# AliBahri94/GM3D

Hardware: AMD Instinct MI355X
Metric: point-clouds/sec pretrain step (N=1024,G=64) (higher is better)
Workload: dtype bf16

## Files before the change

### gm3d_amd/_capi.py

```python
import ctypes
import os

_HERE = os.path.dirname(os.path.abspath(__file__))
LIB_PATH = os.environ.get("GM3D_HIP_LIB") or os.path.join(_HERE, "lib", "libgm3d_hip.so")

GM3D_OK, GM3D_EINVAL, GM3D_EUNSUPPORTED, GM3D_ELAUNCH = 0, -1, -2, -3
GM3D_F32, GM3D_BF16 = 0, 1

_vp, _i, _f = ctypes.c_void_p, ctypes.c_int, ctypes.c_float

SIGNATURES = {
    "gm3d_abi_version": [],
    "gm3d_strerror": [_i],
    "gm3d_fps": [_vp, _i, _i, _i, _vp, _vp, _vp],
    "gm3d_gather_points": [_vp, _vp, _i, _i, _i, _i, _vp, _vp],
    "gm3d_gather_points_grad": [_vp, _vp, _i, _i, _i, _i, _vp, _vp],
    "gm3d_knn": [_vp, _vp, _i, _i, _i, _i, _vp, _vp, _vp],
    "gm3d_knn_group": [_vp, _vp, _i, _i, _i, _i, _vp, _vp, _vp, _vp],
    "gm3d_chamfer_fwd": [_vp, _vp, _i, _i, _i, _vp, _vp, _vp, _vp, _vp],
    "gm3d_chamfer_bwd": [_vp, _vp, _vp, _vp, _vp, _vp, _i, _i, _i, _vp, _vp, _vp],
    "gm3d_patch_chamfer_loss_fwd": [_vp, ctypes.c_longlong, _vp, _vp, ctypes.c_longlong, _i, _i, _i, _vp, _vp, _vp, _vp, _i, _vp],
    "gm3d_patch_chamfer_loss_bwd": [_vp, ctypes.c_longlong, _vp, _vp, ctypes.c_longlong, _vp, _vp, _vp, _i, _i, _i, _vp, _i, _vp],
    "gm3d_attention_fwd": [_vp, _vp, _vp, _i, _i, _i, _f, _i, _vp],
    "gm3d_attention_qkv_fwd": [_vp, _vp, _vp, _vp, _vp, _i, _i, _i, _i, _f, _i, _vp],
    "gm3d_attention_bwd": [_vp, _vp, _vp, _vp, _vp, _i, _i, _i, _f, _i, _vp],
    "gm3d_ln_plain_partial_rows": [_i],
    "gm3d_ln_plain_fwd": [_vp, _vp, _vp, _f, _vp, _vp, _vp, _i, _i, _i, _vp],
    "gm3d_ln_plain_bwd": [_vp, _vp, _vp, _vp, _vp, _vp, _vp, _i, _i, _i, _vp],
    "gm3d_residual_ln_fwd": [_vp, _vp, _vp, _vp, _i, _vp, _vp, _vp, _f, _vp, _vp, _vp, _vp, _i, _i, _i, _vp],
    "gm3d_residual_ln_bwd": [_vp, _vp, _vp, _vp, _vp, _vp, _vp, _i, _vp, _vp, _vp, _vp, _vp, _i, _i, _i, _vp],
    "gm3d_ln_partial_rows": [_i],
    "gm3d_colsum_finish": [_vp, _i, _i, _i, _vp, _i, _vp],
    "gm3d_colsum_finish_batched": [_vp, _i, ctypes.c_longlong, _i, _i, _i, _vp, _i, _vp],
    "gm3d_bias_gelu_fwd": [_vp, _vp, _vp, _i, _i, _i, _vp],
    "gm3d_bias_gelu_bwd": [_vp, _vp, _vp, _vp, _vp, _i, _i, _i, _vp],
    "gm3d_gelu_partial_rows": [_i],
    "gm3d_embed_partial_rows": [_i, _i, _i],
    "gm3d_moments3": [_vp, _i, _vp, _vp],
    "gm3d_pn_layer1_fwd": [_vp, _vp, _vp, _vp, _i, _i, _i, _vp],
    "gm3d_group_max_fwd": [_vp, _vp, _vp, _vp, _i, _i, _i, _i, _vp],
    "gm3d_group_max_bwd": [_vp, _vp, _vp, _i, _i, _i, _i, _vp],
    "gm3d_bn_bcast_stats": [_vp, _vp, _i, _i, _i, _vp, _i, _vp],
    "gm3d_bn_bcast_apply_relu": [_vp, _vp, _vp, _vp, _vp, _i, _i, _i, _f, _i, _vp],
    "gm3d_bn_bcast_bwd_stats": [_vp, _vp, _vp, _vp, _vp, _vp, _vp, _i, _i, _i, _vp, _f, _i, _vp],
    "gm3d_bn_bcast_bwd_apply": [_vp, _vp, _vp, _vp, _vp, _vp, _vp, _vp, _vp, _vp, _vp, _i, _i, _i, _f, _i, _vp],
    "gm3d_head_fold": [_vp, _vp, _i, _i, _vp, _vp, _vp, _i, _vp],
    "gm3d_head_rowdot": [_vp, _vp, _vp, _i, _i, _vp, _i, _vp],
    "gm3d_head_fold_bwd": [_vp, _vp, _i, _i, _i, _vp, _vp, _vp],
    "gm3d_head_outer": [_vp, _vp, _i, _i, _vp, _i, _vp],
    "gm3d_scale_translate": [_vp, _vp, _f, _f, _f, _i, _i, _vp],
    "gm3d_group_select_maps": [_vp, _i, _i, _i, _i, _vp, _vp, _vp],
    "gm3d_bn_bcast_apply_relu_sel": [_vp, _vp, _vp, _vp, _vp, _vp, _i, _i, _i, _f, _i, _vp],
    "gm3d_bn_bcast_bwd_stats_sel": [_vp, _vp, _vp, _vp, _vp, _vp, _vp, _vp, _i, _i, _i, _vp, _f, _i, _vp],
    "gm3d_bn_bcast_bwd_apply_sel": [_vp, _vp, _vp, _vp, _vp, _vp, _vp, _vp, _vp, _vp, _vp, _vp, _i, _i, _i, _f, _i, _vp],
    "gm3d_lin3_gelu_fwd": [_vp, _vp, _vp, _vp, _i, _i, _i, _vp],
    "gm3d_lin3_gelu_bwd": [_vp, _vp, _vp, _vp, _i, _i, _vp, _i, _vp],
    "gm3d_lin3_finish": [_vp, _i, _i, _vp, _vp, _vp],
    "gm3d_rank_loss": [_vp, _vp, _i, _i, _vp, _vp, _vp],
    "gm3d_rank_loss_tail": [_vp, _i, _vp, _i, _i, _vp, _vp, _vp, _vp, _vp],
    "gm3d_rank_loss_tail_bwd": [_vp, _vp, _vp, _i, _i, _i, _vp, _vp],
    "gm3d_ema_counters": [_vp, _vp, _i, _f, _f, _vp],
    "gm3d_drop_path_scales": [_vp, _vp, _i, _i, _vp, _vp],
    "gm3d_pad_cols": [_vp, ctypes.c_longlong, _i, _i, _vp, _i, _i, _vp],
    "gm3d_patch_chamfer_loss_bwd_full": [_vp, ctypes.c_longlong, _vp, _vp, ctypes.c_longlong, _vp, _vp, _vp, _i, _i, _i, _i, _vp, _i, _vp],
    "gm3d_mask_select_b": [_vp, _vp, _i, _i, _i, _i, _vp, _vp, _vp, _vp, _i, _vp],
    "gm3d_pn1_bwd_finalize": [_vp, _vp, _vp, _vp, _vp, _vp, _vp, _vp, _i, _vp],
    "gm3d_gemm_tn_bf16": [_vp, _vp, _vp, _vp, _i, _i, _i, _i, _i, _i, _vp],
    "gm3d_gemm_tn_bf16_gelu": [_vp, _vp, _vp, _vp, _vp, _i, _i, _i, _i, _i, _i, _i, _vp],
    "gm3d_gemm_tn_bf16_pool": [_vp, _vp, _vp, _vp, _vp, _vp, _i, _i, _i, _i, _i, _i, _i, _i, _vp],
    "gm3d_gemm_tn_bf16_gelu_bwd": [_vp, _vp, _vp, _vp, _vp, _vp, _i, _i, _i, _i, _i, _i, _i, _vp],
    "gm3d_gemm_tn_bf16_res": [_vp, _vp, _vp, _vp, _vp, _i, _vp, _vp, _vp, _vp, _i, _i, _i, _i, _i, _i, _vp],
    "gm3d_gemm_tn_bf16_lna": [_vp, _vp, _vp, _vp, _f, _vp, _vp, _vp, _vp, _vp, _vp, _vp, _i, _i, _i, _i, _i, _i, _i, _vp],
    "gm3d_gemm_tile_rows": [_i],
    "gm3d_gemm_tn_bf16_ring": [_vp, _vp, _vp, _vp, _i, _i, _i, _i, _i, _i, _i, _vp],
    "gm3d_gemm_tn_bf16_ws": [_vp, _vp, _vp, _vp, _i, _i, _i, _i, _i, _i, _vp],
    "gm3d_gemm_tn_bf16_ws_pool": [_vp, _vp, _vp, _vp, _vp, _vp, _i, _i, _i, _i, _i, _i, _i, _i, _vp],
    "gm3d_gemm_ws_supported": [_i, _i, _i],
    "gm3d_gemm_tn_bf16_ws_poolg": [_vp, _vp, _vp, _vp, _vp, _vp, _i, _i, _i, _i, _i, _i, _i, _i, _i, _vp],
    "gm3d_gemm_nt_bf16_sum": [_vp, _vp, _vp, _vp, _vp, _i, _i, _i, _i, _i, _i, _i, ctypes.c_longlong, ctypes.c_longlong, ctypes.c_longlong, _i, _vp],
    "gm3d_gemm_nt_tiles": [_i, _i],
    "gm3d_gemm_nt_bf16_multi": [_i] + [_vp] * 14 + [_vp],
    "gm3d_gemm_tn_bf16_ws_bn_apply": [_vp, _vp, _vp, _vp, _vp, _f, _vp, _i, _i, _i, _i, _i, _i, _i, _vp],
    "gm3d_gemm_tn_bf16_ws_bn_stats": [_vp, _vp, _vp, _vp, _vp, _i, _i, _i, _i, _i, _i, _i, _vp],
    "gm3d_gemm_ws_stats_rows": [_i, _i, _i],
    "gm3d_gemm_tn_bf16_ws_bn_apply_g": [_vp, _vp, _vp, _vp, _vp, _f, _vp, _i, _i, _i, _i, _i, _i, _i, _i, _vp],
    "gm3d_gemm_tn_bf16_ws_bn_stats_g": [_vp, _vp, _vp, _vp, _vp, _i, _i, _i, _i, _i, _i, _i, _i, _vp],
    "gm3d_gemm_tn_bf16_ring96": [_vp, _vp, _vp, _vp, _i, _i, _i, _i, _i, _i, _i, _vp],
    "gm3d_gemm_tn_bf16_dma": [_vp, _vp, _vp, _vp, _i, _i, _i, _i, _i, _i, _i, _vp],
    "gm3d_gemm_tn_bf16_dma_gelu_bwd": [_vp, _vp, _vp, _vp, _vp, _vp, _i, _i, _i, _i, _i, _i, _i, _i, _vp],
    "gm3d_gemm_tn_bf16_dma_gelu": [_vp, _vp, _vp, _vp, _vp, _i, _i, _i, _i, _i, _i, _i, _i, _vp],
    "gm3d_transpose_bf16_batched": [_vp, _vp, _i, _i, _i, ctypes.c_longlong, _vp],
    "gm3d_transpose_bf16_multi": [_i, _vp, _vp, _vp, _vp, _vp, _vp, _vp],
    "gm3d_token_assemble_fwd": [_vp, _vp, _vp, _i, _i, _i, _i, _vp, _vp, _vp, _i, _vp],
    "gm3d_token_assemble_bwd": [_vp, _vp, _vp, _vp, _i, _i, _i, _i, _vp, _vp, _i, _vp],
    "gm3d_sum_few_rows": [_vp, _i, _i, ctypes.c_longlong, _vp, _vp],
    "gm3d_gemm_nt_bf16": [_vp, _vp, _vp, _i, _i, _i, _i, _i, _i, _i, ctypes.c_longlong, ctypes.c_longlong, ctypes.c_longlong, _i,
                          ctypes.c_longlong, _vp],
    "gm3d_gemm_nt_bf16_big": [_vp, _vp, _vp, _i, _i, _i, _i, _i, _i, _i, ctypes.c_longlong, ctypes.c_longlong, ctypes.c_longlong, _i,
                              ctypes.c_longlong, _vp],
    "gm3d_gemm_nt_splits": [_i, _i, _i, _i],
    "gm3d_radius_mask_bits": [_vp, _vp, _f, _i, _i, _vp, _vp],
    "gm3d_radius_mask_bits_m": [_vp, _vp, _i, _f, _i, _i, _vp, _vp],
    "gm3d_attention_masked_fwd": [_vp, _vp, _vp, _vp, _i, _i, _i, _i, _f, _i, _vp],
    "gm3d_attention_masked_bwd": [_vp, _vp, _vp, _vp, _vp, _vp, _i, _i, _i, _i, _f, _i, _vp],
    "gm3d_mask_select": [_vp, _vp, _i, _i, _i, _i, _vp, _vp, _vp, _i, _vp],
    "gm3d_bn_finalize": [_vp, ctypes.c_double, _vp, _vp, _f, _f, _vp, _vp, _vp, _vp, _vp, _vp, _vp, _i, _i, _vp],
    "gm3d_pn1_finalize": [_vp, ctypes.c_double, _vp, _vp, _vp, _vp, _f, _f, _vp, _vp, _vp, _vp, _vp, _vp, _vp, _vp, _vp, _i, _i, _vp],
    "gm3d_flat_partial_rows": [ctypes.c_longlong],
    "gm3d_adamw_ema_flat_step": [_vp, _vp, _vp, _vp, _vp, _vp, _vp, ctypes.c_longlong, ctypes.c_longlong, _vp, _f, _f, _f, _f,
                                 _vp, _f, _vp, _vp, _vp, _vp],
    "gm3d_adamw_ema_flat_step_lrd": [_vp, _vp, _vp, _vp, _vp, _vp, _vp, ctypes.c_longlong, ctypes.c_longlong, _vp, _vp, _f, _f,
                                     _f, _f, _vp, _f, _vp, _vp, _vp, _vp],
    "gm3d_group_scatter_add": [_vp, _vp, _vp, _i, _i, _i, _vp, _i, _vp],
    "gm3d_pn_layer1_bwd_stats": [_vp, _vp, _vp, _vp, _vp, _vp, _vp, _vp, _i, _i, _vp, _i, _vp],
    "gm3d_colsum_finish_f64": [_vp, _i, _i, _i, _vp, _vp],
    "gm3d_colsum_partial": [_vp, _i, _i, _vp, _i, _vp],
    "gm3d_gather_inverse": [_vp, _i, _i, _i, _vp, _vp, _vp],
    "gm3d_gather_rows_bwd": [_vp, _vp, _vp, _vp, _i, _i, _i, _i, _i, _vp],
    "gm3d_add_ln_fwd": [_vp, _vp, _vp, _vp, _i, _vp, _vp, _vp, _f, _vp, _vp, _vp, _vp, _i, _i, _i, _vp],
    "gm3d_add_ln_bwd": [_vp, _vp, _vp, _vp, _vp, _vp, _vp, _i, _vp, _vp, _vp, _i, _i, _i, _i, _vp],
    "gm3d_add_ln_bwd_acc": [_vp, _vp, _vp, _vp, _vp, _vp, _vp, _i, _vp, _vp, _vp, _i, _vp, _i, _i, _i, _i, _vp],
    "gm3d_partition_visible": [_vp, _i, _i, _i, _vp, _vp, _vp, _vp, _vp, _vp, _vp],
    "gm3d_select_rows": [_vp, _vp, _vp, _vp, _i, _i, _i, _i, _i, _vp],
    "gm3d_back_project": [_vp, _vp, _i, _i, _i, _i, _vp, _vp],
    "gm3d_interp3_fwd": [_vp, _vp, _vp, _vp, _vp, _i, _i, _i, _i, _i, _i, _vp],
    "gm3d_gather_rows_bwd_w": [_vp, _i, _i, _i, _vp, _vp, _vp, _vp, _i, _i, _i, _i, _i, _vp],
    "gm3d_where_rows": [_vp, _i, _vp, _vp, _i, _vp, ctypes.c_longlong, _i, _i, _vp],
    "gm3d_take_rows": [_vp, _vp, _vp, _i, _i, _i, _i, _i, _vp],
    "gm3d_colsum_partial_w": [_vp, _vp, _i, _i, _vp, _i, _vp],
    "gm3d_gemm_tn_bf16_dma_pool": [_vp, _vp, _vp, _vp, _vp, _vp, _i, _i, _i, _i, _i, _i, _i, _i, _i, _i, _vp],
    "gm3d_gemm_tn_bf16_dmaw": [_vp, _vp, _vp, _vp, _i, _i, _i, _i, _i, _i, _i, _i, _vp],
    "gm3d_vote_sample": [_vp, _vp, _vp, _vp, _vp, _i, _i, _i, _i, _i, _vp, _vp],
    "gm3d_cls_tail_vote": [_vp, _i, _i, _i, _i] + [_vp] * 14 + [_i, _f, _vp, _vp, _vp, _vp, _vp, _i, _vp],
    "gm3d_cls_tail_fwd": [_vp, _i, _i, _i, _i] + [_vp] * 10 + [_i] + [_vp] * 6 + [_f, _f, _i] + [_vp] * 8 + [_i, _vp],
    "gm3d_cls_tail_bwd": [_i, _i, _i, _i] + [_vp] * 7 + [_i, _i] + [_vp] * 21 + [_i, _vp],
    "gm3d_cls_tail_vote_pool": [_vp, _i, _i, _i, _i, _i] + [_vp] * 14 + [_i, _f, _vp, _vp, _vp, _vp, _vp, _vp, _i, _vp],
    "gm3d_svm_gram": [_vp, _i, _i, _vp, _vp],
    "gm3d_svm_smo": [_vp, _i, _i, _vp, ctypes.c_double, ctypes.c_double, ctypes.c_longlong, _vp, _vp, _vp, _vp, _vp],
    "gm3d_svm_weights": [_vp, _i, _i, _i, _vp, _vp, _vp, _vp],
    "gm3d_svm_predict": [_vp, _i, _i, _i, _vp, _vp, _vp, _vp, _vp, _vp],
}


class Gm3dError(RuntimeError):
    pass


def _load():
    if not os.path.exists(LIB_PATH):
        raise ImportError(
            "gm3d_amd: %s not found. Build it with `python -m gm3d_amd.build` "
            "(hipcc, --offload-arch=gfx950). There is no CPU fallback." % LIB_PATH)
    lib = ctypes.CDLL(LIB_PATH)
    for name, argtypes in SIGNATURES.items():
        fn = getattr(lib, name)
        fn.argtypes = argtypes
        fn.restype = ctypes.c_char_p if name == "gm3d_strerror" else ctypes.c_int
    return lib


lib = _load()


def check(rc, what):
    if rc != GM3D_OK:
        raise Gm3dError("%s failed: %s (code %d)" % (what, lib.gm3d_strerror(rc).decode(), rc))
```

### gm3d_amd/build.py

```python
import glob
import os
import subprocess
import sys

HERE = os.path.dirname(os.path.abspath(__file__))
CSRC = os.path.join(HERE, "csrc")
OUT_DIR = os.path.join(HERE, "lib")
LIB = os.path.join(OUT_DIR, "libgm3d_hip.so")
ARCH = "gfx950"

SOURCES = {
    "capi.hip": [],
    "fps.hip": ["-ffp-contract=off"],
    "knn.hip": ["-ffp-contract=off"],
    "chamfer.hip": ["-ffp-contract=off"],
    "attention.hip": [],
    "rowops.hip": [],
    "embed.hip": [],
    "optim.hip": [],
    "gemm.hip": [],
    "gemm_nt.hip": [],
    "gemm_ring.hip": [],
    "gemm_dma.hip": [],
    "gemm_ws.hip": [],
    "gather.hip": [],
    "attention_masked.hip": [],
    "vote.hip": [],
    "cls_tail.hip": [],
    "svm.hip": ["-ffp-contract=off"],
}
COMMON = ["--offload-arch=" + ARCH, "-O3", "-fPIC", "-std=c++17", "-Wall", "-Wno-unused-function"]


def _stale(target, deps):
    if not os.path.exists(target):
        return True
    t = os.path.getmtime(target)
    return any(os.path.getmtime(d) > t for d in deps)


def build(force=False, verbose=False):
    hipcc = os.environ.get("HIPCC", "/opt/rocm/bin/hipcc")
    os.makedirs(OUT_DIR, exist_ok=True)
    hdrs = sorted(glob.glob(os.path.join(CSRC, "*.hpp"))) + [os.path.join(HERE, "..", "include", "gm3d.h")]
    objs = []
    for src, extra in SOURCES.items():
        s = os.path.join(CSRC, src)
        o = os.path.join(OUT_DIR, src.replace(".hip", ".o"))
        if force or _stale(o, [s] + hdrs):
            cmd = [hipcc] + COMMON + extra + ["-c", s, "-o", o]
            if verbose:
                print(" ".join(cmd))
            subprocess.check_call(cmd)
        objs.append(o)
    if force or _stale(LIB, objs):
        cmd = [hipcc, "--offload-arch=" + ARCH, "-shared", "-fPIC", "-o", LIB] + objs
        if verbose:
            print(" ".join(cmd))
        subprocess.check_call(cmd)
    return LIB


if __name__ == "__main__":
    print(build(force="--force" in sys.argv, verbose=True))
```

### gm3d_amd/embed.py

```python
import torch

from ._capi import lib
from .fused import weight_cache, LNC
from . import gemm
from .ops import _launch, _ptr, _stream, _DT

SPLITK = 64


def _finish(partial, nrows, ncols, pitch=None):
    out = torch.empty(ncols, dtype=torch.float32, device=partial.device)
    _launch("gm3d_colsum_finish", {"rows": nrows, "cols": ncols}, lib.gm3d_colsum_finish, _ptr(partial), nrows,
            pitch or ncols, ncols, _ptr(out), 0, _stream())
    return out


def colsum(m, adt):
    R, C = m.shape
    nrows = lib.gm3d_embed_partial_rows(2, R, C)
    partial = torch.empty(nrows, C, dtype=torch.float32, device=m.device)
    _launch("gm3d_colsum_partial", {"R": R, "C": C, "dtype": str(m.dtype)}, lib.gm3d_colsum_partial, _ptr(m), R, C,
            _ptr(partial), _DT[m.dtype], _stream())
    return _finish(partial, nrows, C)


def splitk_wgrad(dy, x):
    R, N = dy.shape
    K = x.shape[1]
    from . import gemm
    if dy.is_contiguous() and x.is_contiguous() and gemm.wgrad_supported(dy.unsqueeze(0), x.unsqueeze(0)):
        return gemm.wgrad_nt(dy.unsqueeze(0), x.unsqueeze(0))[0]
    if (N % 128 and N < 128 and dy.is_contiguous() and x.is_contiguous() and dy.dtype == torch.bfloat16
            and gemm.wgrad_supported(dy.new_empty(1, R, 128), x.unsqueeze(0))):
        pad = torch.zeros(R, 128, dtype=dy.dtype, device=dy.device)
        pad[:, :N] = dy
        return gemm.wgrad_nt(pad.unsqueeze(0), x.unsqueeze(0))[0][:N].contiguous()
    S = SPLITK if R % SPLITK == 0 and R >= 64 * SPLITK else 1
    a = dy.view(S, R // S, N).transpose(1, 2)
    b = x.view(S, R // S, K)
    if dy.dtype == torch.float32:
        part = torch.bmm(a, b)
    else:
        try:
            part = torch.bmm(a, b, out_dtype=torch.float32)
        except TypeError:
            part = torch.bmm(a, b).float()
    if S == 1:
        return part[0]
    from . import fused
    if not fused.SUM_FEW_ROWS:
        return _finish(part.view(S, N * K), S, N * K).view(N, K)
    out = torch.empty(N, K, dtype=torch.float32, device=dy.device)
    _launch("gm3d_sum_few_rows", {"rows": S, "cols": N * K}, lib.gm3d_sum_few_rows, _ptr(part), 1, S, N * K, _ptr(out), _stream())
    return out


def _c32(p):
    p = p.detach()
    return p if (p.dtype == torch.float32 and p.is_contiguous()) else p.float().contiguous()


class EmbedFn(torch.autograd.Function):

    @staticmethod
    def forward(ctx, nb, meta, w1, b1, g1, be1, w2, b2, w3, b3, g2, be2, w4, b4, rm1, rv1, nbt1, rm2, rv2, nbt2):
        with torch.autocast("cuda", enabled=False):
            return EmbedFn._forward(ctx, nb, meta, w1, b1, g1, be1, w2, b2, w3, b3, g2, be2, w4, b4, rm1, rv1, nbt1,
                                    rm2, rv2, nbt2)

    @staticmethod
    def _forward(ctx, nb, meta, w1, b1, g1, be1, w2, b2, w3, b3, g2, be2, w4, b4, rm1, rv1, nbt1, rm2, rv2, nbt2):
        adt, training, eps, mom = meta["adt"], meta["training"], meta["eps"], meta["momentum"]
        dt_id = _DT[adt]
        B, G, K, _ = nb.shape
        BG, R = B * G, B * G * K
        dev = nb.device
        x = nb.reshape(R, 3).float().contiguous()
        C1, C2, C3, C4 = w1.shape[0], w2.shape[0], w3.shape[0], w4.shape[0]
        W1 = w1.reshape(C1, 3)
        f64 = torch.float64
        f32 = dict(dtype=torch.float32, device=dev)
        mom9 = mcov = xmean = None
        if training:
            nrows = lib.gm3d_embed_partial_rows(0, R, 0)
            part = torch.empty(nrows, 9, dtype=f64, device=dev)
            _launch("gm3d_moments3", {"R": R}, lib.gm3d_moments3, _ptr(x), R, _ptr(part), _stream())
            mom9 = torch.empty(9, dtype=f64, device=dev)
            _launch("gm3d_colsum_finish_f64", {"rows": nrows, "cols": 9}, lib.gm3d_colsum_finish_f64, _ptr(part), nrows, 9, 9,
                    _ptr(mom9), _stream())
            mcov = torch.empty(12, dtype=f64, device=dev)
            xmean = torch.empty(3, **f32)
        w1c, b1c, g1c, be1c = _c32(W1), _c32(b1), _c32(g1), _c32(be1)
        wf, bf = torch.empty(C1, 3, **f32), torch.empty(C1, **f32)
        mean1, rstd1 = torch.empty(C1, **f32), torch.empty(C1, **f32)
        _launch("gm3d_pn1_finalize", {"C": C1}, lib.gm3d_pn1_finalize, _ptr(mom9), float(R), _ptr(w1c), _ptr(b1c), _ptr(g1c),
                _ptr(be1c), eps, mom, _ptr(rm1), _ptr(rv1), _ptr(nbt1), _ptr(wf), _ptr(bf), _ptr(mean1), _ptr(rstd1),
                _ptr(mcov), _ptr(xmean), C1, int(training), _stream())
        a1 = torch.empty(R, C1, dtype=adt, device=dev)
        _launch("gm3d_pn_layer1_fwd", {"R": R, "C": C1, "dtype": str(adt)}, lib.gm3d_pn_layer1_fwd, _ptr(x), _ptr(wf),
                _ptr(bf), _ptr(a1), R, C1, dt_id, _stream())
        W2 = weight_cache.get(w2, adt).reshape(C2, C1)
        pool_fused = gemm.FUSE_POOL and ((K == 32 and gemm.supported(a1, W2)) or (K == 16 and gemm.pool16_supported(a1, W2)))
        if pool_fused:
            f, fg, arg1 = gemm.linear_pool(a1, W2, _c32(b2), bias_after_pool=False, want_rows=True, group_rows=K)
        else:
            f = gemm.mm(a1, W2, _c32(b2)) if adt == torch.bfloat16 else torch.addmm(weight_cache.get(b2, adt), a1, W2.t())
            fg = torch.empty(BG, C2, dtype=adt, device=dev)
            arg1 = torch.empty(BG, C2, dtype=torch.uint8, device=dev)
            _launch("gm3d_group_max_fwd", {"G": BG, "K": K, "C": C2, "dtype": str(adt)}, lib.gm3d_group_max_fwd, _ptr(f), None,
                    _ptr(fg), _ptr(arg1), BG, K, C2, dt_id, _stream())
        W3 = weight_cache.get(w3, adt).reshape(C3, 2 * C2)
        W3g, W3l = W3[:, :C2], W3[:, C2:]
        t = gemm.mm(fg, W3g, _c32(b3))
        vis = meta.get("vis_ids")
        fuse_bn = K in (16, 32) and gemm.ws_bn_supported(f, W3l, t, group_rows=K)
        y0 = st = None
        if training:
            if fuse_bn and (K == 32 or gemm.WS_BN_STATS16):
                y0, part = gemm.linear_ws_bn_stats(f, W3l, t, group_rows=K)
                st = _finish(part, part.shape[0], 2 * C3)
            else:
                y0 = gemm.mm(f, W3l)
                nrows = lib.gm3d_embed_partial_rows(1, BG, C3)
                part = torch.empty(nrows, 2 * C3, dtype=torch.float32, device=dev)
                _launch("gm3d_bn_bcast_stats", {"G": BG, "K": K, "C": C3, "dtype": str(adt)}, lib.gm3d_bn_bcast_stats, _ptr(y0),
                        _ptr(t), BG, K, C3, _ptr(part), dt_id, _stream())
                st = _finish(part, nrows, 2 * C3)
        g2c, be2c = _c32(g2), _c32(be2)
        scale2, shift2 = torch.empty(C3, **f32), torch.empty(C3, **f32)
        mean2, rstd2 = torch.empty(C3, **f32), torch.empty(C3, **f32)
        _launch("gm3d_bn_finalize", {"C": C3}, lib.gm3d_bn_finalize, _ptr(st), float(R), _ptr(g2c), _ptr(be2c), eps, mom,
                _ptr(rm2), _ptr(rv2), _ptr(nbt2), _ptr(scale2), _ptr(shift2), _ptr(mean2), _ptr(rstd2), C3, int(training),
                _stream())
        sel = inv = None
        BGs, Gs = BG, G
        if vis is not None:
            if vis.dim() != 2 or vis.shape[0] != B or vis.dtype != torch.int64 or vis.stride(1) != 1 or vis.shape[1] > G:
                raise ValueError("vis_ids must be (B,V) int64 with unit inner stride, V <= G")
            Gs = vis.shape[1]
            BGs = B * Gs
            sel = torch.empty(BGs, dtype=torch.int32, device=dev)
            inv = torch.empty(BG, dtype=torch.int32, device=dev)
            _launch("gm3d_group_select_maps", {"B": B, "V": Gs, "G": G}, lib.gm3d_group_select_maps, _ptr(vis), vis.stride(0), B,
                    Gs, G, _ptr(sel), _ptr(inv), _stream())
        if not training and fuse_bn and vis is None:
            a2 = gemm.linear_ws_bn_apply(f, W3l, t, scale2, shift2, group_rows=K)
        else:
            if y0 is None:
                y0 = gemm.mm(f, W3l)
            a2 = torch.empty(BGs * K, C3, dtype=adt, device=dev)
            _launch("gm3d_bn_bcast_apply_relu", {"G": BGs, "K": K, "C": C3, "dtype": str(adt)}, lib.gm3d_bn_bcast_apply_relu_sel,
                    _ptr(y0), _ptr(t), _ptr(scale2), _ptr(shift2), _ptr(a2), _ptr(sel), BGs, K, C3, 0.0, dt_id, _stream())
        W4 = weight_cache.get(w4, adt).reshape(C4, C3)
        b4f = _c32(b4)
        if gemm.FUSE_POOL and ((K == 32 and gemm.supported(a2, W4)) or (K == 16 and gemm.pool16_supported(a2, W4))):
            _, tok, arg2 = gemm.linear_pool(a2, W4, b4f, bias_after_pool=True, want_rows=False, group_rows=K)
        else:
            z = gemm.mm(a2, W4) if adt == torch.bfloat16 else a2 @ W4.t()
            tok = torch.empty(BGs, C4, dtype=adt, device=dev)
            arg2 = torch.empty(BGs, C4, dtype=torch.uint8, device=dev)
            _launch("gm3d_group_max_fwd", {"G": BGs, "K": K, "C": C4, "dtype": str(adt)}, lib.gm3d_group_max_fwd, _ptr(z),
                    _ptr(b4f), _ptr(tok), _ptr(arg2), BGs, K, C4, dt_id, _stream())
        if meta["grad"] and any(ctx.needs_input_grad):
            if not training:
                raise NotImplementedError("EmbedFn backward is implemented for train-mode BatchNorm only")
            ctx.save_for_backward(x, a1, f, fg, arg1, y0, t, a2, arg2, w1, b1, g1, w2, w3, g2, w4, mcov, xmean,
                                  mean1, rstd1, mean2, rstd2, scale2, shift2)
            ctx.meta, ctx.dims = meta, (B, G, K, C1, C2, C3, C4)
            ctx.sel, ctx.inv, ctx.Gs = sel, inv, Gs
        return tok.view(B, Gs, C4)

    @staticmethod
    def backward(ctx, dtok):
        with torch.autocast("cuda", enabled=False):
            return EmbedFn._backward(ctx, dtok)

    @staticmethod
    def _backward(ctx, dtok):
        (x, a1, f, fg, arg1, y0, t, a2, arg2, w1, b1, g1, w2, w3, g2, w4, mcov, xmean, mean1, rstd1, mean2, rstd2, scale2,
         shift2) = ctx.saved_tensors
        adt = ctx.meta["adt"]
        dt_id = _DT[adt]
        B, G, K, C1, C2, C3, C4 = ctx.dims
        BG, R = B * G, B * G * K
        dev = dtok.device
        f64 = torch.float64
        sel, inv, BGs = ctx.sel, ctx.inv, B * ctx.Gs
        dtok = dtok.reshape(BGs, C4).to(adt).contiguous()
        db4 = colsum(dtok, adt)
        dz = torch.empty(BGs * K, C4, dtype=adt, device=dev)
        _launch("gm3d_group_max_bwd", {"G": BGs, "K": K, "C": C4, "dtype": str(adt)}, lib.gm3d_group_max_bwd, _ptr(dtok),
                _ptr(arg2), _ptr(dz), BGs, K, C4, dt_id, _stream())
        W4 = weight_cache.get(w4, adt).reshape(C4, C3)
        da2 = gemm.mm_nn(dz, W4)
        later = []
        multi = gemm.MULTI_WGRAD and adt == torch.bfloat16 and gemm.ENABLED

        def wgrad(dy_, x_):
            if multi and dy_.is_contiguous() and x_.is_contiguous() and gemm.wgrad_multi_ok(dy_.unsqueeze(0), x_.unsqueeze(0), None):
                out = torch.empty(1, dy_.shape[1], x_.shape[1], dtype=torch.float32, device=dev)
                later.append((dy_.unsqueeze(0), x_.unsqueeze(0), out))
                return out[0]
            return splitk_wgrad(dy_, x_)
        dW4 = wgrad(dz, a2)
        nrows = lib.gm3d_embed_partial_rows(1, BGs, C3)
        part = torch.empty(nrows, 2 * C3, dtype=torch.float32, device=dev)
        _launch("gm3d_bn_bcast_bwd_stats", {"G": BGs, "K": K, "C": C3, "dtype": str(adt)}, lib.gm3d_bn_bcast_bwd_stats_sel,
                _ptr(da2), _ptr(y0), _ptr(t), _ptr(scale2), _ptr(shift2), _ptr(mean2), _ptr(rstd2), _ptr(sel), BGs, K, C3,
                _ptr(part), 0.0, dt_id, _stream())
        s12 = _finish(part, nrows, 2 * C3)
        s1, s2 = s12[:C3], s12[C3:]
        dy = torch.empty(R, C3, dtype=adt, device=dev)
        dt = torch.empty(BG, C3, dtype=torch.float32, device=dev)
        _launch("gm3d_bn_bcast_bwd_apply", {"G": BG, "K": K, "C": C3, "dtype": str(adt)}, lib.gm3d_bn_bcast_bwd_apply_sel,
                _ptr(da2), _ptr(y0), _ptr(t), _ptr(scale2), _ptr(shift2), _ptr(mean2), _ptr(rstd2), _ptr(s1), _ptr(s2),
                _ptr(dy), _ptr(dt), _ptr(inv), BG, K, C3, 0.0, dt_id, _stream())
        dg2, dbe2 = s2, s1
        W3 = weight_cache.get(w3, adt).reshape(C3, 2 * C2)
        W3g, W3l = W3[:, :C2], W3[:, C2:]
        bf16 = adt == torch.bfloat16 and gemm.ENABLED
        if bf16:
            W3T = gemm.transposed(W3)
        df = gemm.mm(dy, W3T[C2:]) if bf16 else dy @ W3l
        dW3l = wgrad(dy, f)
        db3 = colsum(dt, torch.float32)
        dta = dt.to(adt)
        dW3g = wgrad(dta, fg)
        dfg = gemm.mm(dta, W3T[:C2]) if bf16 else dta @ W3g
        nrows = lib.gm3d_embed_partial_rows(1, BG, C2)
        part = torch.empty(nrows, C2, dtype=torch.float32, device=dev)
        _launch("gm3d_group_scatter_add", {"G": BG, "K": K, "C": C2, "dtype": str(adt)}, lib.gm3d_group_scatter_add, _ptr(df),
                _ptr(dfg), _ptr(arg1), BG, K, C2, _ptr(part), dt_id, _stream())
        db2 = _finish(part, nrows, C2)
        W2 = weight_cache.get(w2, adt).reshape(C2, C1)
        da1 = gemm.mm_nn(df, W2)
        dW2 = wgrad(df, a1).reshape(w2.shape)
        W1 = _c32(w1.reshape(C1, 3))
        nrows = lib.gm3d_embed_partial_rows(4, R, C1)
        part = torch.empty(nrows, 5 * C1, dtype=f64, device=dev)
        b1f, g1f = _c32(b1), _c32(g1)
        _launch("gm3d_pn_layer1_bwd_stats", {"R": R, "C": C1, "dtype": str(adt)}, lib.gm3d_pn_layer1_bwd_stats, _ptr(da1),
                _ptr(a1), _ptr(x), _ptr(W1), _ptr(b1f), _ptr(mean1), _ptr(rstd1), _ptr(xmean), R, C1, _ptr(part), dt_id,
                _stream())
        q = torch.empty(5 * C1, dtype=f64, device=dev)
        _launch("gm3d_colsum_finish_f64", {"rows": nrows, "cols": 5 * C1}, lib.gm3d_colsum_finish_f64, _ptr(part), nrows,
                5 * C1, 5 * C1, _ptr(q), _stream())
        dW1 = torch.empty(C1, 3, dtype=torch.float32, device=dev)
        dg1, dbe1 = torch.empty(C1, dtype=torch.float32, device=dev), torch.empty(C1, dtype=torch.float32, device=dev)
        _launch("gm3d_pn1_bwd_finalize", {"C": C1}, lib.gm3d_pn1_bwd_finalize, _ptr(q), _ptr(mcov), _ptr(W1), _ptr(g1f),
                _ptr(rstd1), _ptr(dW1), _ptr(dg1), _ptr(dbe1), C1, _stream())
        db1 = torch.zeros_like(b1)
        if len(later) > 1:
            gemm.wgrad_nt_multi(later)
        elif later:
            gemm.wgrad_nt(later[0][0], later[0][1], later[0][2])
        dW3 = torch.cat([dW3g, dW3l], dim=1).reshape(w3.shape)
        return (None, None, dW1.reshape(w1.shape), db1, dg1, dbe1, dW2, db2, dW3, db3, dg2, dbe2,
                dW4.reshape(w4.shape), db4, None, None, None, None, None, None)


def run_embed(enc, point_groups, vis_ids=None):
    c0, bn0, _, c1 = enc.first_conv
    c2, bn1, _, c3 = enc.second_conv
    adt = torch.bfloat16 if (torch.is_autocast_enabled() and torch.get_autocast_dtype("cuda") == torch.bfloat16) \
        else torch.float32
    meta = {"adt": adt, "training": enc.training, "eps": bn0.eps, "momentum": bn0.momentum,
            "grad": torch.is_grad_enabled(), "vis_ids": vis_ids}
    return EmbedFn.apply(point_groups, meta, c0.weight, c0.bias, bn0.weight, bn0.bias, c1.weight, c1.bias, c2.weight,
                         c2.bias, bn1.weight, bn1.bias, c3.weight, c3.bias, bn0.running_mean, bn0.running_var,
                         bn0.num_batches_tracked, bn1.running_mean, bn1.running_var, bn1.num_batches_tracked)
```

### include/gm3d.h

```cpp
#ifndef GM3D_H
#define GM3D_H
#include <stdint.h>

#ifdef __cplusplus
extern "C" {
#endif

typedef void *gm3d_stream_t;

enum {
    GM3D_OK = 0,
    GM3D_EINVAL = -1,
    GM3D_EUNSUPPORTED = -2,
    GM3D_ELAUNCH = -3
};

enum { GM3D_F32 = 0, GM3D_BF16 = 1 };

int gm3d_abi_version(void);
const char *gm3d_strerror(int code);

int gm3d_fps(const float *xyz, int B, int N, int npoint, int32_t *idx, float *centers,
             gm3d_stream_t stream);

int gm3d_gather_points(const float *feat, const int32_t *idx, int B, int C, int N, int M,
                       float *out, gm3d_stream_t stream);

int gm3d_gather_points_grad(const float *grad_out, const int32_t *idx, int B, int C, int N, int M,
                            float *grad_feat, gm3d_stream_t stream);

int gm3d_knn(const float *ref, const float *query, int B, int N, int G, int k,
             float *dist, int64_t *idx, gm3d_stream_t stream);

int gm3d_knn_group(const float *xyz, const float *center, int B, int N, int G, int k,
                   int64_t *idx, float *neighborhood, float *neighborhood_org,
                   gm3d_stream_t stream);

int gm3d_chamfer_fwd(const float *xyz1, const float *xyz2, int P, int n, int m,
                     float *dist1, float *dist2, int32_t *idx1, int32_t *idx2,
                     gm3d_stream_t stream);

int gm3d_chamfer_bwd(const float *xyz1, const float *xyz2, const int32_t *idx1, const int32_t *idx2,
                     const float *grad_dist1, const float *grad_dist2, int P, int n, int m,
                     float *gxyz1, float *gxyz2, gm3d_stream_t stream);

int gm3d_attention_fwd(const void *qkv, void *out, float *lse, int B, int T, int H,
                       float scale, int dtype, gm3d_stream_t stream);

int gm3d_attention_qkv_fwd(const void *h, const void *wqkv, void *out, float *lse, void *qkv_out,
                           int B, int T, int H, int C, float scale, int dtype, gm3d_stream_t stream);

int gm3d_attention_bwd(const void *qkv, const void *out, const void *dout, const float *lse,
                       void *dqkv, int B, int T, int H, float scale, int dtype,
                       gm3d_stream_t stream);

int gm3d_patch_chamfer_loss_fwd(const void *pred, long long pred_bstride, const float *target, const long long *ids,
                                long long ids_bstride, int B, int T, int M, float *matrix, int32_t *idx1, int32_t *idx2,
                                float *mean_out, int dtype, gm3d_stream_t stream);
int gm3d_patch_chamfer_loss_bwd(const void *pred, long long pred_bstride, const float *target, const long long *ids,
                                long long ids_bstride, const int32_t *idx1, const int32_t *idx2, const float *gmean, int B, int T,
                                int M, void *dpred, int dtype, gm3d_stream_t stream);
int gm3d_patch_chamfer_loss_bwd_full(const void *pred, long long pred_bstride, const float *target, const long long *ids,
                                     long long ids_bstride, const int32_t *idx1, const int32_t *idx2, const float *gmean, int B, int T,
                                     int M, int lead, void *dpred, int dtype, gm3d_stream_t stream);

int gm3d_ln_plain_partial_rows(int R);
int gm3d_ln_plain_fwd(const void *x, const float *gamma, const float *beta, float eps, void *h, float *mean, float *rstd, int R,
                      int C, int dtype, gm3d_stream_t stream);
int gm3d_ln_plain_bwd(const void *dh, const void *x, const float *mean, const float *rstd, const float *gamma, void *dx,
                      float *partial, int R, int C, int dtype, gm3d_stream_t stream);
int gm3d_add_ln_fwd(const void *x, const void *y, const float *ybias, const float *rowscale, int rows_per_sample, const void *z,
                    const float *gamma, const float *beta, float eps, void *s_out, void *h, float *mean, float *rstd, int R, int C,
                    int dtype, gm3d_stream_t stream);
int gm3d_add_ln_bwd(const void *dh, const void *gin, const void *x, const float *mean, const float *rstd, const float *gamma,
                    const float *rowscale, int rows_per_sample, void *dx, void *dy, float *partial, int nsum, int R, int C, int dtype,
                    gm3d_stream_t stream);
int gm3d_add_ln_bwd_acc(const void *dh, const void *gin, const void *x, const float *mean, const float *rstd, const float *gamma,
                        const float *rowscale, int rows_per_sample, void *dx, void *dy, float *partial, int nsum, void *acc,
                        int acc_mode, int R, int C, int dtype, gm3d_stream_t stream);


int gm3d_residual_ln_fwd(const float *res, const void *y, const float *bias, const float *rowscale,
                         int rows_per_sample, const void *add, const float *gamma, const float *beta,
                         float eps, float *out_res, void *h, float *mean, float *rstd, int R, int C,
                         int dtype, gm3d_stream_t stream);

int gm3d_residual_ln_bwd(const void *dh, const float *gin, const float *x, const float *mean,
                         const float *rstd, const float *gamma, const float *rowscale, int rows_per_sample,
                         float *dx, void *dy, float *acc, void *acc_out, float *partial, int R, int C, int dtype,
                         gm3d_stream_t stream);
int gm3d_ln_partial_rows(int R);

int gm3d_colsum_finish(const float *partial, int nrows, int pitch, int ncols, float *out, int accumulate,
                       gm3d_stream_t stream);

int gm3d_colsum_finish_batched(const float *partial, int njobs, long long job_stride, int nrows, int pitch, int ncols,
                               float *out, int out_stride, gm3d_stream_t stream);

int gm3d_bias_gelu_fwd(const void *f, const float *bias, void *g, int R, int C, int dtype,
                       gm3d_stream_t stream);
int gm3d_bias_gelu_bwd(const void *dg, const void *f, const float *bias, void *df, float *partial, int R,
                       int C, int dtype, gm3d_stream_t stream);
int gm3d_gelu_partial_rows(int R);

int gm3d_embed_partial_rows(int kind, int n, int C);

int gm3d_moments3(const float *x, int R, double *partial, gm3d_stream_t stream);

int gm3d_pn_layer1_fwd(const float *x, const float *wf, const float *bf, void *a1, int R, int C1, int dtype,
                       gm3d_stream_t stream);

int gm3d_group_max_fwd(const void *in, const float *bias, void *out, uint8_t *arg, int G, int K, int C, int dtype,
                       gm3d_stream_t stream);
int gm3d_group_max_bwd(const void *dout, const uint8_t *arg, void *din, int G, int K, int C, int dtype,
                       gm3d_stream_t stream);

int gm3d_bn_bcast_stats(const void *y0, const void *t, int G, int K, int C, float *partial, int dtype,
                        gm3d_stream_t stream);
int gm3d_bn_bcast_apply_relu(const void *y0, const void *t, const float *scale, const float *shift, void *a2,
                             int G, int K, int C, float slope, int dtype, gm3d_stream_t stream);
int gm3d_bn_bcast_bwd_stats(const void *da2, const void *y0, const void *t, const float *scale, const float *shift,
                            const float *mean, const float *rstd, int G, int K, int C, float *partial, float slope,
                            int dtype, gm3d_stream_t stream);
int gm3d_bn_bcast_bwd_apply(const void *da2, const void *y0, const void *t, const float *scale, const float *shift,
                            const float *mean, const float *rstd, const float *s1, const float *s2, void *dy,
                            float *dt, int G, int K, int C, float slope, int dtype, gm3d_stream_t stream);

int gm3d_head_fold(const float *W1, const float *b1, int nout, int C, float *wv, void *wv_t, float *bm, int dtype,
                   gm3d_stream_t stream);
int gm3d_head_rowdot(const void *a, const void *wv_t, const float *bm, int R, int C, float *out, int dtype, gm3d_stream_t stream);
int gm3d_head_fold_bwd(const float *dwv, const float *d, int R, int nout, int C, float *dW1, float *db1, gm3d_stream_t stream);
int gm3d_head_outer(const float *d, const float *wv, int R, int C, void *da, int dtype, gm3d_stream_t stream);

int gm3d_scale_translate(float *pc, const float *u, float lo, float span, float t, int B, int N, gm3d_stream_t stream);

int gm3d_group_select_maps(const long long *ids, int id_pitch, int B, int V, int G, int *sel, int *inv, gm3d_stream_t stream);
int gm3d_bn_bcast_apply_relu_sel(const void *y0, const void *t, const float *scale, const float *shift, void *a2,
                                 const int *sel, int G, int K, int C, float slope, int dtype, gm3d_stream_t stream);
int gm3d_bn_bcast_bwd_stats_sel(const void *da2, const void *y0, const void *t, const float *scale, const float *shift,
                                const float *mean, const float *rstd, const int *sel, int G, int K, int C, float *partial,
                                float slope, int dtype, gm3d_stream_t stream);
int gm3d_bn_bcast_bwd_apply_sel(const void *da2, const void *y0, const void *t, const float *scale, const float *shift,
                                const float *mean, const float *rstd, const float *s1, const float *s2, void *dy, float *dt,
                                const int *inv, int G, int K, int C, float slope, int dtype, gm3d_stream_t stream);

int gm3d_group_scatter_add(void *df, const void *dfg, const uint8_t *arg, int G, int K, int C, float *partial,
                           int dtype, gm3d_stream_t stream);

int gm3d_pn_layer1_bwd_stats(const void *da1, const void *a1, const float *x, const float *w1, const float *b1,
                             const float *mean, const float *rstd, const float *xmean, int R, int C1,
                             double *partial, int dtype, gm3d_stream_t stream);
int gm3d_colsum_finish_f64(const double *partial, int nrows, int pitch, int ncols, double *out,
                           gm3d_stream_t stream);

int gm3d_colsum_partial(const void *m, int R, int C, float *partial, int dtype, gm3d_stream_t stream);
int gm3d_colsum_partial_w(const void *m, const float *roww, int R, int C, float *partial, int dtype, gm3d_stream_t stream);

int gm3d_lin3_gelu_fwd(const float *x, const float *w, const float *b, void *out, int R, int C, int dtype,
                       gm3d_stream_t stream);
int gm3d_lin3_gelu_bwd(const void *dout, const float *x, const float *w, const float *b, int R, int C,
                       double *partial, int dtype, gm3d_stream_t stream);
int gm3d_lin3_finish(const double *partial, int nrows, int C, float *dW, float *db, gm3d_stream_t stream);

int gm3d_rank_loss(const float *pred, const float *target, int B, int M, float *out, float *dpred,
                   gm3d_stream_t stream);
int gm3d_rank_loss_tail(const float *pred, int ldp, const float *target, int B, int M, float *out, float *dpred, float *tot, float *loss,
                        gm3d_stream_t stream);
int gm3d_rank_loss_tail_bwd(const float *dpred, const float *g, const float *tot, int B, int M, int L, float *dfull, gm3d_stream_t stream);
int gm3d_ema_counters(long long *e, const long long *m, int n, float decay, float w, gm3d_stream_t stream);
int gm3d_drop_path_scales(const float *u, const float *keep, int S, int B, float *out, gm3d_stream_t stream);
int gm3d_pad_cols(const void *src, long long lds, int R, int N, void *dst, int Np, int dtype, gm3d_stream_t stream);

int gm3d_flat_partial_rows(long long n);
int gm3d_adamw_ema_flat_step(float *params, const float *grads, float *exp_avg, float *exp_avg_sq, float *ema,
                             void *shadow_p, void *shadow_e, long long n, long long n_decay, const float *lr_dev,
                             float weight_decay, float beta1, float beta2, float eps, const float *ema_w_dev,
                             float max_norm, float *step_dev, float *partial, float *scal, gm3d_stream_t stream);
int gm3d_adamw_ema_flat_step_lrd(float *params, const float *grads, float *exp_avg, float *exp_avg_sq, float *ema,
                                 void *shadow_p, void *shadow_e, long long n, long long n_decay, const float *lr_dev,
                                 const float *lr_scale, float weight_decay, float beta1, float beta2, float eps,
                                 const float *ema_w_dev, float max_norm, float *step_dev, float *partial, float *scal,
                                 gm3d_stream_t stream);

int gm3d_bn_finalize(const float *sums, double rows, const float *gamma, const float *beta, float eps, float momentum,
                     float *running_mean, float *running_var, long long *nbt, float *scale, float *shift,
                     float *mean_out, float *rstd_out, int C, int training, gm3d_stream_t stream);
int gm3d_pn1_finalize(const double *mom9, double rows, const float *w, const float *b, const float *gamma,
                      const float *beta, float eps, float momentum, float *running_mean, float *running_var,
                      long long *nbt, float *wf, float *bf, float *mean_out, float *rstd_out, double *mcov,
                      float *xmean, int C, int training, gm3d_stream_t stream);
int gm3d_pn1_bwd_finalize(const double *q, const double *mcov, const float *w, const float *gamma, const float *rstd,
                          float *dw, float *dgamma, float *dbeta, int C, gm3d_stream_t stream);
int gm3d_mask_select(const float *loss_pred, const float *noise, int B, int L, int len_keep, int len_loss, float *mask,
                     long long *vis_ids, long long *mask_ids, int id_pitch, gm3d_stream_t stream);
int gm3d_mask_select_b(const float *loss_pred, const float *noise, int B, int L, int len_keep, int len_loss, float *mask,
                       unsigned char *mask_bool, long long *vis_ids, long long *mask_ids, int id_pitch, gm3d_stream_t stream);
int gm3d_gemm_tn_bf16(const void *A, const void *W, const float *bias, void *C, int M, int N, int K, int lda, int ldw,
                      int ldc, gm3d_stream_t stream);
int gm3d_gemm_tn_bf16_gelu(const void *A, const void *W, const float *bias, void *F, void *G, int M, int N, int K, int lda,
                           int ldw, int ldf, int ldg, gm3d_stream_t stream);
int gm3d_gemm_tn_bf16_pool(const void *A, const void *W, const float *bias, void *C, void *P, uint8_t *arg, int M, int N, int K,
                           int lda, int ldw, int ldc, int ldp, int bias_after_pool, gm3d_stream_t stream);
int gm3d_gemm_tn_bf16_gelu_bwd(const void *dO, const void *Wt, const void *F, const float *bias, void *dF, float *colpart, int M,
                               int N, int K, int lda, int ldw, int ldf, int lddf, gm3d_stream_t stream);
int gm3d_gemm_tn_bf16_res(const void *A, const void *W, const float *bias, const float *res, const float *rowscale, int rows_per_sample,
                          const void *add, float *U, void *U16, float *stats, int M, int N, int K, int lda, int ldw, int bm,
                          gm3d_stream_t stream);
int gm3d_gemm_tn_bf16_lna(const void *U16, const float *stats, const float *gamma, const float *beta, float eps, const void *W,
                          const float *bias, void *C, void *G, void *H, float *mean, float *rstd, int M, int N, int K, int ldu, int ldw,
                          int ldc, int ldg, gm3d_stream_t stream);
int gm3d_gemm_tile_rows(int M);
int gm3d_gemm_tn_bf16_ring(const void *A, const void *W, const float *bias, void *C, int M, int N, int K, int lda, int ldw, int ldc,
                           int bm, gm3d_stream_t stream);
int gm3d_gemm_tn_bf16_ws(const void *A, const void *W, const float *bias, void *C, int M, int N, int K, int lda, int ldw, int ldc,
                         gm3d_stream_t stream);
int gm3d_gemm_tn_bf16_ws_pool(const void *A, const void *W, const float *bias, void *C, void *P, unsigned char *arg, int M, int N, int K,
                              int lda, int ldw, int ldc, int ldp, int bias_after_pool, gm3d_stream_t stream);
int gm3d_gemm_tn_bf16_ws_poolg(const void *A, const void *W, const float *bias, void *C, void *P, unsigned char *arg, int M, int N, int K,
                               int lda, int ldw, int ldc, int ldp, int bias_after_pool, int group_rows, gm3d_stream_t stream);
int gm3d_gemm_ws_supported(int N, int K, int pool);
int gm3d_gemm_tn_bf16_ws_bn_apply(const void *A, const void *W, const void *T, const float *scale, const float *shift, float slope, void *C,
                                  int M, int N, int K, int lda, int ldw, int ldt, int ldc, gm3d_stream_t stream);
int gm3d_gemm_tn_bf16_ws_bn_stats(const void *A, const void *W, const void *T, void *C, float *partial, int M, int N, int K, int lda,
                                  int ldw, int ldt, int ldc, gm3d_stream_t stream);
int gm3d_gemm_tn_bf16_ws_bn_apply_g(const void *A, const void *W, const void *T, const float *scale, const float *shift, float slope, void *C,
                                    int M, int N, int K, int lda, int ldw, int ldt, int ldc, int group_rows, gm3d_stream_t stream);
int gm3d_gemm_tn_bf16_ws_bn_stats_g(const void *A, const void *W, const void *T, void *C, float *partial, int M, int N, int K, int lda,
                                    int ldw, int ldt, int ldc, int group_rows, gm3d_stream_t stream);
int gm3d_gemm_ws_stats_rows(int M, int N, int K);
int gm3d_gemm_tn_bf16_ring96(const void *A, const void *W, const float *bias, void *C, int M, int N, int K, int lda, int ldw, int ldc,
                             int bm, gm3d_stream_t stream);
int gm3d_gemm_tn_bf16_dma(const void *A, const void *W, const float *bias, void *C, int M, int N, int K, int lda, int ldw, int ldc,
                          int bm, gm3d_stream_t stream);
int gm3d_gemm_tn_bf16_dmaw(const void *A, const void *W, const float *bias, void *C, int M, int N, int K, int lda, int ldw, int ldc,
                           int bm, int bn, gm3d_stream_t stream);
int gm3d_gemm_tn_bf16_dma_pool(const void *A, const void *W, const float *bias, void *C, void *P, unsigned char *arg, int M, int N,
                               int K, int lda, int ldw, int ldc, int ldp, int bias_after_pool, int bm, int bn, gm3d_stream_t stream);
int gm3d_gemm_tn_bf16_dma_gelu(const void *A, const void *W, const float *bias, void *F, void *G, int M, int N, int K, int lda,
                               int ldw, int ldf, int ldg, int bm, gm3d_stream_t stream);
int gm3d_gemm_tn_bf16_dma_gelu_bwd(const void *dO, const void *Wt, const void *F, const float *bias, void *dF, float *colpart, int M,
                                   int N, int K, int lda, int ldw, int ldf, int lddf, int bm, gm3d_stream_t stream);
int gm3d_transpose_bf16_batched(const void *src, void *dst, int batch, int rows, int cols, long long src_batch_stride,
                                gm3d_stream_t stream);
int gm3d_transpose_bf16_multi(int count, const void *const *src, void *const *dst, const int *batch, const int *rows, const int *cols,
                              const long long *src_batch_stride, gm3d_stream_t stream);
int gm3d_token_assemble_fwd(const void *tokens, const void *pos, const long long *order, int B, int L, int V, int C, void *x_vis,
                            void *pos_vis, void *pos_full, int dtype, gm3d_stream_t stream);
int gm3d_token_assemble_bwd(const void *dx_vis, const void *dpos_vis, const void *dpos_full, const long long *order, int B, int L,
                            int V, int C, void *dtokens, void *dpos, int dtype, gm3d_stream_t stream);
int gm3d_sum_few_rows(const float *partial, int njobs, int nrows, long long ncols, float *out, gm3d_stream_t stream);
int gm3d_gemm_nt_bf16(const void *dY, const void *X, float *out, int batch, int R, int N, int K, int ldy, int ldx, int ldo,
                      long long stride_y, long long stride_x, long long stride_o, int splits, long long stride_split,
                      gm3d_stream_t stream);
int gm3d_gemm_nt_splits(int batch, int R, int N, int K);
int gm3d_gemm_nt_bf16_big(const void *dY, const void *X, float *out, int batch, int R, int N, int K, int ldy, int ldx, int ldo,
                          long long stride_y, long long stride_x, long long stride_o, int splits, long long stride_split,
                          gm3d_stream_t stream);
int gm3d_gemm_nt_bf16_sum(const void *dY, const void *X, float *part, float *out, int *counters, int batch, int R, int N, int K, int ldy,
                          int ldx, int ldo, long long stride_y, long long stride_x, long long stride_o, int splits, gm3d_stream_t stream);
int gm3d_gemm_nt_tiles(int N, int K);
int gm3d_gemm_nt_bf16_multi(int count, const void *const *dY, const void *const *X, float *const *out, float *const *part, const int *batch,
                            const int *R, const int *N, const int *K, const int *ldy, const int *ldx, const long long *stride_y,
                            const long long *stride_x, const long long *stride_o, const int *splits, gm3d_stream_t stream);
int gm3d_gather_inverse(const long long *idx, int B, int J, int S, int *off, int *list, gm3d_stream_t stream);
int gm3d_gather_rows_bwd(const void *dy, const int *off, const int *list, void *dx, int B, int J, int S, int C, int dtype,
                         gm3d_stream_t stream);
int gm3d_radius_mask_bits(const float *center, const unsigned char *vis, float radius, int B, int G, unsigned *bits,
                          gm3d_stream_t stream);
// ... 58 lines not shown
```

Baseline: 17140.

## Compute pooled-layer input gradient sparsely from max-pool argmax instead of dense GEMM

Adds a HIP kernel that computes da2 = dz·W4 by exploiting the fact that dz is nonzero only at argmax positions of the group max-pool. Each wave ballots which output channels map to each row and accumulates only those weight rows held in LDS, skipping the dense GEMM over mostly-zero dz. It is restricted to bf16, C_out=384 and group sizes 16/32. The dense group_max_bwd that produces dz still runs, and the kernel's cost depends on how the argmax indices are distributed.

```diff
diff --git a/gm3d_amd/_capi.py b/gm3d_amd/_capi.py
--- a/gm3d_amd/_capi.py
+++ b/gm3d_amd/_capi.py
@@ -40,6 +40,7 @@
     "gm3d_pn_layer1_fwd": [_vp, _vp, _vp, _vp, _i, _i, _i, _vp],
     "gm3d_group_max_fwd": [_vp, _vp, _vp, _vp, _i, _i, _i, _i, _vp],
     "gm3d_group_max_bwd": [_vp, _vp, _vp, _i, _i, _i, _i, _vp],
+    "gm3d_pool_input_grad": [_vp, _vp, _vp, _vp, _i, _i, _i, _i, _i, _vp],
     "gm3d_bn_bcast_stats": [_vp, _vp, _i, _i, _i, _vp, _i, _vp],
     "gm3d_bn_bcast_apply_relu": [_vp, _vp, _vp, _vp, _vp, _i, _i, _i, _f, _i, _vp],
     "gm3d_bn_bcast_bwd_stats": [_vp, _vp, _vp, _vp, _vp, _vp, _vp, _i, _i, _i, _vp, _f, _i, _vp],
diff --git a/gm3d_amd/build.py b/gm3d_amd/build.py
--- a/gm3d_amd/build.py
+++ b/gm3d_amd/build.py
@@ -17,6 +17,7 @@
     "attention.hip": [],
     "rowops.hip": [],
     "embed.hip": [],
+    "pool_grad.hip": [],
     "optim.hip": [],
     "gemm.hip": [],
     "gemm_nt.hip": [],
diff --git a/gm3d_amd/csrc/pool_grad.hip b/gm3d_amd/csrc/pool_grad.hip
--- /dev/null
+++ b/gm3d_amd/csrc/pool_grad.hip
@@ -0,0 +1,94 @@
+#include "common.hpp"
+
+namespace gm3d {
+
+constexpr int PG_CO = 384, PG_SLOTS = PG_CO / 64, PG_COLS = 128, PG_WAVES = 16, PG_ROWS = 8, PG_GRID_Y = 64;
+
+__device__ __forceinline__ float pg_lo(unsigned w) { return __builtin_bit_cast(float, w << 16); }
+__device__ __forceinline__ float pg_hi(unsigned w) { return __builtin_bit_cast(float, w & 0xffff0000u); }
+
+__device__ __forceinline__ void pg_take(unsigned long long& m, float d, const unsigned* wslot, float& v, unsigned& w) {
+    const int b = __builtin_ctzll(m);
+    m &= m - 1;
+    v = __builtin_bit_cast(float, __builtin_amdgcn_readlane(__builtin_bit_cast(int, d), b));
+    w = wslot[b * 64];
+}
+
+template <int Q>
+__global__ __launch_bounds__(PG_WAVES * 64) void pool_input_grad_kernel(const bf16_t* __restrict__ dtok, const uint8_t* __restrict__ arg,
+                                                                        const bf16_t* __restrict__ W, bf16_t* __restrict__ dx, int groups,
+                                                                        int C_in) {
+    extern __shared__ unsigned pg_w[];
+    const int col0 = blockIdx.x * PG_COLS;
+    for (int p = threadIdx.x; p < PG_CO * 16; p += PG_WAVES * 64) {
+        const int c = p >> 4, q = p & 15;
+        *reinterpret_cast<uint4*>(pg_w + c * 64 + q * 4) = *reinterpret_cast<const uint4*>(W + (size_t)c * C_in + col0 + q * 8);
+    }
+    __syncthreads();
+    const int lane = threadIdx.x & 63;
+    const int wave = __builtin_amdgcn_readfirstlane((int)(threadIdx.x >> 6));
+    const int K = Q * PG_ROWS, items = groups * Q;
+    const unsigned* wl = pg_w + lane;
+    for (int it = blockIdx.y * PG_WAVES + wave; it < items; it += gridDim.y * PG_WAVES) {
+        const int g = it / Q, r0 = (it % Q) * PG_ROWS;
+        int a[PG_SLOTS];
+        float d[PG_SLOTS];
+#pragma unroll
+        for (int s = 0; s < PG_SLOTS; ++s) {
+            a[s] = arg[(size_t)g * PG_CO + s * 64 + lane];
+            d[s] = (float)dtok[(size_t)g * PG_CO + s * 64 + lane];
+        }
+        unsigned* out = reinterpret_cast<unsigned*>(dx + ((size_t)g * K + r0) * C_in + col0) + lane;
+        const size_t pitch = (size_t)C_in / 2;
+        for (int j = 0; j < PG_ROWS / 2; ++j) {
+            const int ra = r0 + j, rb = ra + PG_ROWS / 2;
+            float a0 = 0.f, a1 = 0.f, b0 = 0.f, b1 = 0.f;
+#pragma unroll
+            for (int s = 0; s < PG_SLOTS; ++s) {
+                unsigned long long ma = __ballot(a[s] == ra), mb = __ballot(a[s] == rb);
+                const unsigned* ws = wl + s * 64 * 64;
+                float va, vb;
+                unsigned wa, wb;
+                while (ma && mb) {
+                    pg_take(ma, d[s], ws, va, wa);
+                    pg_take(mb, d[s], ws, vb, wb);
+                    a0 = fmaf(va, pg_lo(wa), a0); a1 = fmaf(va, pg_hi(wa), a1);
+                    b0 = fmaf(vb, pg_lo(wb), b0); b1 = fmaf(vb, pg_hi(wb), b1);
+                }
+                while (ma) {
+                    pg_take(ma, d[s], ws, va, wa);
+                    a0 = fmaf(va, pg_lo(wa), a0); a1 = fmaf(va, pg_hi(wa), a1);
+                }
+                while (mb) {
+                    pg_take(mb, d[s], ws, vb, wb);
+                    b0 = fmaf(vb, pg_lo(wb), b0); b1 = fmaf(vb, pg_hi(wb), b1);
+                }
+            }
+            out[(size_t)j * pitch] = (unsigned)__builtin_bit_cast(unsigned short, (bf16_t)a0)
+                                   | ((unsigned)__builtin_bit_cast(unsigned short, (bf16_t)a1) << 16);
+            out[(size_t)(j + PG_ROWS / 2) * pitch] = (unsigned)__builtin_bit_cast(unsigned short, (bf16_t)b0)
+                                                   | ((unsigned)__builtin_bit_cast(unsigned short, (bf16_t)b1) << 16);
+        }
+    }
+}
+
+}
+
+extern "C" int gm3d_pool_input_grad(const void* dtok, const uint8_t* arg, const void* W, void* dx, int groups, int group_rows, int C_out,
+                                    int C_in, int dtype, gm3d_stream_t stream) {
+    using namespace gm3d;
+    if (!dtok || !arg || !W || !dx || groups < 1 || group_rows < 1 || C_out < 1 || C_in < 1) return GM3D_EINVAL;
+    if (dtype != GM3D_F32 && dtype != GM3D_BF16) return GM3D_EINVAL;
+    if (dtype != GM3D_BF16 || (group_rows != 32 && group_rows != 16) || C_out != PG_CO || C_in % PG_COLS != 0) return GM3D_EUNSUPPORTED;
+    if (groups > (1 << 26)) return GM3D_EUNSUPPORTED;
+    const int q = group_rows / PG_ROWS;
+    const long long items = (long long)groups * q;
+    const int gy = (int)((items + PG_WAVES - 1) / PG_WAVES < PG_GRID_Y ? (items + PG_WAVES - 1) / PG_WAVES : PG_GRID_Y);
+    const dim3 grid(C_in / PG_COLS, gy), block(PG_WAVES * 64);
+    const size_t lds = (size_t)PG_CO * 64 * sizeof(unsigned);
+    if (q == 4)
+        return launch_lds<pool_input_grad_kernel<4>>(grid, block, lds, stream, (const bf16_t*)dtok, arg, (const bf16_t*)W, (bf16_t*)dx,
+                                                     groups, C_in);
+    return launch_lds<pool_input_grad_kernel<2>>(grid, block, lds, stream, (const bf16_t*)dtok, arg, (const bf16_t*)W, (bf16_t*)dx,
+                                                 groups, C_in);
+}
diff --git a/gm3d_amd/embed.py b/gm3d_amd/embed.py
--- a/gm3d_amd/embed.py
+++ b/gm3d_amd/embed.py
@@ -52,6 +52,25 @@
         return _finish(part.view(S, N * K), S, N * K).view(N, K)
     out = torch.empty(N, K, dtype=torch.float32, device=dy.device)
     _launch("gm3d_sum_few_rows", {"rows": S, "cols": N * K}, lib.gm3d_sum_few_rows, _ptr(part), 1, S, N * K, _ptr(out), _stream())
+    return out
+
+
+POOL_INPUT_GRAD = True
+
+
+def pool_input_grad_supported(dtok, arg, w, group_rows):
+    return (POOL_INPUT_GRAD and gemm.ENABLED and dtok.is_cuda and dtok.dtype == torch.bfloat16 and w.dtype == torch.bfloat16
+            and group_rows in (16, 32) and w.shape[0] == 384 and w.shape[1] % 128 == 0 and dtok.is_contiguous() and arg.is_contiguous()
+            and w.is_contiguous() and w.data_ptr() % 16 == 0 and arg.dtype == torch.uint8 and dtok.shape == arg.shape)
+
+
+def pool_input_grad(dtok, arg, w, group_rows, out=None):
+    G, C_out = dtok.shape
+    C_in = w.shape[1]
+    if out is None:
+        out = torch.empty(G * group_rows, C_in, dtype=dtok.dtype, device=dtok.device)
+    _launch("gm3d_pool_input_grad", {"G": G, "K": group_rows, "C_out": C_out, "C_in": C_in}, lib.gm3d_pool_input_grad, _ptr(dtok), _ptr(arg),
+            _ptr(w), _ptr(out), G, group_rows, C_out, C_in, _DT[dtok.dtype], _stream())
     return out
 
 
@@ -192,7 +211,10 @@
         _launch("gm3d_group_max_bwd", {"G": BGs, "K": K, "C": C4, "dtype": str(adt)}, lib.gm3d_group_max_bwd, _ptr(dtok),
                 _ptr(arg2), _ptr(dz), BGs, K, C4, dt_id, _stream())
         W4 = weight_cache.get(w4, adt).reshape(C4, C3)
-        da2 = gemm.mm_nn(dz, W4)
+        if pool_input_grad_supported(dtok, arg2, W4, K):
+            da2 = pool_input_grad(dtok, arg2, W4, K)
+        else:
+            da2 = gemm.mm_nn(dz, W4)
         later = []
         multi = gemm.MULTI_WGRAD and adt == torch.bfloat16 and gemm.ENABLED
 
diff --git a/include/gm3d.h b/include/gm3d.h
--- a/include/gm3d.h
+++ b/include/gm3d.h
@@ -114,6 +114,8 @@
                        gm3d_stream_t stream);
 int gm3d_group_max_bwd(const void *dout, const uint8_t *arg, void *din, int G, int K, int C, int dtype,
                        gm3d_stream_t stream);
+int gm3d_pool_input_grad(const void *dtok, const uint8_t *arg, const void *W, void *dx, int groups, int group_rows, int C_out,
+                         int C_in, int dtype, gm3d_stream_t stream);
 
 int gm3d_bn_bcast_stats(const void *y0, const void *t, int G, int K, int C, float *partial, int dtype,
                         gm3d_stream_t stream);
```

After: 16980. No clear change (-0.9%).
